# quang-ha/lammps-sph-multiphase

Hardware: AMD Instinct MI355X
Metric: particle-steps/s + achieved HBM GB/s, 1M-particle taitwater+rhosum, 1/2/4/8 GPUs (higher is better)
Workload: dtype f64

## Files before the change

### include/sph_hip.h

```cpp
#ifndef SPH_HIP_H
#define SPH_HIP_H

#include <stdint.h>

#ifdef __cplusplus
extern "C" {
#endif

#define SPH_HIP_ABI_VERSION 2

#define SPH_HIP_OK 0
#define SPH_HIP_EINVAL (-1)
#define SPH_HIP_ENODEV (-2)
#define SPH_HIP_ERUNTIME (-3)
#define SPH_HIP_ENOMEM (-4)
#define SPH_HIP_ECOMM (-5)
#define SPH_HIP_EOVERFLOW (-6)

#define SPH_LIST_FULL 0
#define SPH_LIST_HALF 1

#define SPH_VISC_MONAGHAN 0
#define SPH_VISC_MORRIS 1

// ... 129 lines not shown
  int kernel_path;
  const sph_engine_mp_config *mp;
} sph_engine_config;

typedef struct {
  int64_t step;
  int nlocal, nghost;
  int64_t nbr_full;
  int nbr_builds;
  int nbr_maxrow;
  int staged;
  int stage_max;
  double ms_rhosum, ms_tait, ms_heat, ms_integrate, ms_comm, ms_neigh;
  int64_t n_rhosum, n_tait, n_heat, n_neigh;
  int blk_nbig;
  int inner_rows;
  int inner_live;
  int flags;
  int64_t inner_refresh;
} sph_engine_stats;

#define SPH_STAT_RHO_FUSED (1 << 0)
#define SPH_STAT_BLK_R32 (1 << 1)
#define SPH_STAT_BLK_BIGIMG (1 << 2)
#define SPH_STAT_BLK_NOPRE (1 << 3)
#define SPH_STAT_BLK_ROWRETRY (1 << 4)
#define SPH_STAT_BLK_IMGRETRY (1 << 5)
#define SPH_STAT_MP_W4 (1 << 6)
#define SPH_STAT_MP_POW (1 << 7)
#define SPH_STAT_MP_ROW (1 << 8)
#define SPH_STAT_MP_RHO_LISTFILL (1 << 9)
#define SPH_STAT_CSORT_BINS (1 << 10)
#define SPH_STAT_CSORT_ROWS (1 << 11)

typedef struct sph_engine sph_engine;

int sph_engine_create(int device, const sph_engine_config *cfg, sph_engine **out);
int sph_engine_destroy(sph_engine *e);

int sph_engine_comm_uid(void *uid128);
int sph_engine_comm_init(sph_engine *e, const void *uid128, int nranks, int rank);
int sph_engine_comm_loopback(sph_engine *e, int on);
typedef struct sph_local_world sph_local_world;
int sph_local_world_create(int nranks, sph_local_world **out);
int sph_local_world_destroy(sph_local_world *w);
int sph_engine_comm_local(sph_engine *e, sph_local_world *w, int rank);
int sph_engine_comm_ipc(sph_engine *e, const char *name, int nranks, int rank, int mode);
#define SPH_TUNE_OVERLAP 1
#define SPH_TUNE_BLKUMF 2
#define SPH_TUNE_CSORT 3
int sph_engine_tune(sph_engine *e, int key, int value);
int sph_engine_csort_paths(sph_engine *e, int *mask);
int sph_engine_set_tags(sph_engine *e, const int *tags);

int sph_engine_set_atoms(sph_engine *e, int n, const double *x, const double *v,
                         const int *type, const double *rho, const double *en,
                         const double *cv);
int sph_engine_set_atoms_multiphase(sph_engine *e, const double *rmass, const double *cv,
                                    const double *cg);
int sph_engine_phase_change(sph_engine *e, const sph_phasechange_params *p, int nevery,
                            int seed);
int sph_engine_atom_sort(sph_engine *e, int sortfreq, double binsize);

int sph_engine_neigh_modify(sph_engine *e, int every, int delay, int check);

typedef struct {
  int64_t builds;
  int64_t dangerous;
  int64_t checks;
  int64_t last_build;
} sph_neigh_stats;
int sph_engine_neigh_stats(sph_engine *e, sph_neigh_stats *out);

typedef struct {
  int nevery;
  int minbound; double tmin;
  int maxbound; double tmax;
  double xmax;
  int type_mask;
} sph_dtreset;
int sph_engine_dt_reset(sph_engine *e, const sph_dtreset *fix);

typedef struct {
// ... 130 lines not shown
```

### lammps-sph-multiphase_amd/__init__.py

```python
from __future__ import annotations

import ctypes as C
import os

import numpy as np

HERE = os.path.dirname(os.path.abspath(__file__))
LIB_PATH = os.environ.get("SPH_HIP_LIB") or os.path.join(HERE, "libsph_hip.so")
HEADER = os.path.join(os.path.dirname(HERE), "include", "sph_hip.h")

SPH_LIST_FULL, SPH_LIST_HALF = 0, 1
SPH_VISC_MONAGHAN, SPH_VISC_MORRIS = 0, 1
SPH_MAXTYPES = 8
_NT2 = (SPH_MAXTYPES + 1) ** 2

ERRORS = {-1: "EINVAL", -2: "ENODEV", -3: "ERUNTIME", -4: "ENOMEM", -5: "ECOMM",
          -6: "EOVERFLOW"}


class HipError(RuntimeError):
    def __init__(self, code: int, msg: str):
        super().__init__(f"sph_hip {ERRORS.get(code, code)}: {msg}")
        self.code = code

# ... 856 lines not shown
            for c in classes:
                mask |= 1 << c
            _chk(self.L.sph_engine_set_timing(self.h, mask << 1))
        else:
            _chk(self.L.sph_engine_set_timing(self.h, 1 if on else 0))

    @property
    def nlocal(self):
        return self.L.sph_engine_nlocal(self.h)

    def get_atoms(self):
        n = self.nlocal
        out = {k: np.zeros((n, 3)) for k in ("x", "v", "f")}
        out.update({k: np.zeros(n) for k in ("rho", "e", "drho", "de")})
        out["tag"] = np.zeros(n, dtype=np.int32)
        _chk(self.L.sph_engine_get_atoms(self.h, out["x"].ctypes.data, out["v"].ctypes.data,
                                         out["rho"].ctypes.data, out["e"].ctypes.data,
                                         out["f"].ctypes.data, out["drho"].ctypes.data,
                                         out["de"].ctypes.data, out["tag"].ctypes.data))
        return out

    def set_tags(self, tags):
        tags = np.ascontiguousarray(tags, dtype=np.int32)
        _chk(self.L.sph_engine_set_tags(self.h, tags))

    def comm_local(self, world: "LocalWorld", rank: int):
        _chk(self.L.sph_engine_comm_local(self.h, world.h, rank))
        self._world = world

    def comm_init(self, uid: bytes, nranks: int, rank: int):
        buf = C.create_string_buffer(bytes(uid), 128)
        _chk(self.L.sph_engine_comm_init(self.h, buf, nranks, rank))

    TUNE_OVERLAP, TUNE_BLKUMF, TUNE_CSORT = 1, 2, 3

    def tune(self, key: int, value: int):
        _chk(self.L.sph_engine_tune(self.h, key, int(value)))

    IPC_DEVICE, IPC_HOST = 0, 1

    def comm_ipc(self, name: str, nranks: int, rank: int, mode: int = 0):
        _chk(self.L.sph_engine_comm_ipc(self.h, name.encode(), nranks, rank, int(mode)))

    def comm_loopback(self, on: bool = True):
        _chk(self.L.sph_engine_comm_loopback(self.h, 1 if on else 0))

    def neighbor_counts(self):
        c = np.zeros(self.nlocal, dtype=np.int32)
        _chk(self.L.sph_engine_neighbor_counts(self.h, c))
        return c

    STAT_RHO_FUSED, STAT_BLK_R32, STAT_BLK_BIGIMG = 1 << 0, 1 << 1, 1 << 2
    STAT_BLK_NOPRE, STAT_BLK_ROWRETRY, STAT_BLK_IMGRETRY = 1 << 3, 1 << 4, 1 << 5
    STAT_MP_W4, STAT_MP_POW, STAT_MP_ROW, STAT_MP_RHO_LISTFILL = 1 << 6, 1 << 7, 1 << 8, 1 << 9
    STAT_CSORT_BINS, STAT_CSORT_ROWS = 1 << 10, 1 << 11

    def csort_paths(self) -> int:
        m = _i(0)
        _chk(self.L.sph_engine_csort_paths(self.h, C.byref(m)))
        return m.value

    def stats(self) -> dict:
        s = EngineStats()
        _chk(self.L.sph_engine_stats_get(self.h, C.byref(s)))
        return s.as_dict()


def _moments_dict(count, mass, mx, mv, lo, hi, volume):
    d = dict(count=count, mass=mass, mx=mx, mv=mv, lo=lo, hi=hi, volume=volume)
    d["xcm"] = mx / mass if mass > 0.0 else np.zeros(3)
    d["vcm"] = mv / mass if mass > 0.0 else np.zeros(3)
    return d


def combine_moments(ranks):
    first = ranks[0]
    acc = {k: (first[k].copy() if isinstance(first[k], np.ndarray) else first[k])
           for k in ("count", "mass", "mx", "mv", "lo", "hi", "volume")}
    for r in ranks[1:]:
        for k in ("count", "mass", "mx", "mv", "volume"):
            acc[k] = acc[k] + r[k]
        acc["lo"] = np.minimum(acc["lo"], r["lo"])
        acc["hi"] = np.maximum(acc["hi"], r["hi"])
    return _moments_dict(**acc)


def gyration_dict(sums, mass):
    sums = np.array(sums, dtype=np.float64)
# ... 57 lines not shown
```

### lammps-sph-multiphase_amd/csrc/sph_blk_kernels.h

```cpp
#pragma once
#include <hip/hip_runtime.h>

#include <algorithm>
#include <type_traits>
#include <utility>

#include "sph_engine_kernels.h"
#include "sph_row2_kernels.h"
#include "sph_select.h"
#include "sph_util.h"

namespace sph {

constexpr int BLK_TPR = 16;

template <int BT>
__device__ __forceinline__ int blk_scan(int v, int *s_w, int *total) {
  const int lane = threadIdx.x & 63, w = threadIdx.x >> 6;
  int x = v;
#pragma unroll
  for (int d = 1; d < 64; d <<= 1) {
    const int y = __shfl_up(x, d, 64);
    if (lane >= d) x += y;
  }
// ... 968 lines not shown
      for (int p = tid; p < u; p += NTH)
        if ((s_bm[(p + 1) >> 5] >> ((p + 1) & 31)) & 1u)
          uilist[(size_t)b * ucap + rank(p + 1)] = ul[p];
    if (ren && tid == 0) {
      uicnt[b] = tot;
      if (umax) {
        atomicMax(umax, tot);
        atomicAdd(umax + 1, tot);
      }
    }
    const int grp = (tid & 63) / G;
    unsigned short *const out = snbi + (size_t)rr * sstride;
    int base = 0;
    sw.walk(c, lane, [&](int q, bool in) {
      const bool hit = hit_of(q, in);
      const unsigned long long m = __ballot(hit);
      const unsigned g = (unsigned)(m >> (grp * G)) & ((1u << G) - 1u);
      if (hit)
        out[blk_tpos<G, U>(base + __popc(g & ((1u << lane) - 1u)))] =
            (unsigned short)(ren ? blk_q(rank(blk_s<CQ>(q)) + 1, CQ) : q);
      base += __popc(g);
    });
    if (live) {
      if (lane == 0) {
        icnt[row] = base;
        if (x0) x0[row] = xi;
      }
      const int cend = min((base + U * G - 1) / (U * G) * (U * G), sstride);
      for (int k = base + lane; k < cend; k += G) out[blk_tpos<G, U>(k)] = 0;
    }
  }
}

#define SPH_BLK_FORCE_PARAMS                                                              \
  int n, const int *__restrict__ ulist, const int *__restrict__ ucnt, int ucap,                 \
      const unsigned short *__restrict__ snbr, int sstride, const int *__restrict__ rcnt,     \
      const double4 *__restrict__ xf, const double4 *__restrict__ vr,                         \
      const int *__restrict__ ty, const double *__restrict__ en,                              \
      const Coefs *__restrict__ cf, double4 *__restrict__ fo, double *__restrict__ de,        \
      double gx, double gy, double gz, int um, int cq,                                        \
      const unsigned short *__restrict__ snbi, const int *__restrict__ icnt,                  \
      const int *__restrict__ moved, const int *__restrict__ uilist,                          \
      const int *__restrict__ uicnt, const int *__restrict__ blist
#define SPH_BLK_FORCE_ARGS                                                                \
  n, ulist, ucnt, ucap, snbr, sstride, rcnt, xf, vr, ty, en, cf, fo, de, gx, gy, gz, um, cq, \
      snbi, icnt, moved, uilist, uicnt, blist
template <int R, int G, int U, int NCH, int VISC, int MODE, bool NT1, int EXP = 0, int AHEAD = 1>
__device__ __forceinline__ void blk_force_body(SPH_BLK_FORCE_PARAMS) {
  if (snbi && *moved == 0) {
    snbr = snbi;
    rcnt = icnt;
    ulist = uilist;
    ucnt = uicnt;
  }
  constexpr bool GAS = (MODE & M_GAS) != 0;
  constexpr bool TAIT = (MODE & (M_TAIT | M_GAS)) != 0;
  constexpr bool HEAT = (MODE & M_HEAT) != 0;
  constexpr bool EIMG = HEAT || GAS;
  constexpr int NTH = R * G;
  constexpr int CQ = (EIMG ? BLK_CHE : BLK_CH) / 16;
  constexpr bool FOLDV = TAIT && !HEAT && !GAS && NT1 && VISC == SPH_VISC_MONAGHAN;
  extern __shared__ __attribute__((aligned(16))) unsigned char blk_smem[];
  __shared__ TaitPair s_tp[(TAIT && !NT1) ? NT2 : 1];
  __shared__ HeatPair s_hp[(HEAT && !NT1) ? NT2 : 1];
  const int nt1 = cf->ntypes + 1;
  const int b = blist ? blist[xcd_block()] : (int)xcd_block();
  const int tid = threadIdx.x;
  const int u = EXP == 3 ? 0 : ucnt[b];
  const int nwin = u > um ? (u + um - 1) / um : 1;
  const int u0 = min(u, um);
  const int row = b * R + tid / G, lane = tid & (G - 1);
  const bool live = row < n;
  const int rr = live ? row : n - 1;
  const int c = live ? rcnt[rr] : 0;
  const int *const ul = ulist + (size_t)b * ucap;
  int jj[BLK_SP];
#pragma unroll
  for (int k = 0; k < BLK_SP; k++) jj[k] = tid + k * NTH < u0 ? ul[tid + k * NTH] : -1;
  BlkSlots<G, U, NCH> sw;
  sw.load(snbr + (size_t)rr * sstride, c, lane);
  const double4 xi = xf[rr];
// ... 139 lines not shown
  auto walk = [&](auto ld) {
    if constexpr (NCH > 0)
      blk_walk3<AHEAD>(sw, wave_max_count<G>(c), ld, pair);
    else
      sw.walk(c, lane, [&](int q, bool) { pair(ld(q)); });
  };
  if (nwin == 1) {
    walk(load);
  } else {
    const int qmax = blk_q(um, CQ);
    for (int w = 0; w < nwin; w++) {
      if (w > 0) {
        __syncthreads();
        stage(w, tid);
        __syncthreads();
      }
      const int qo = blk_q(w * um, CQ);
      walk([&](int q) {
        const int qq = q - qo;
        return load((unsigned)(qq - 1) < (unsigned)qmax ? qq : 0);
      });
    }
  }
  if (TAIT) {
    fx = group_sum<G>(fx);
    fy = group_sum<G>(fy);
    fz = group_sum<G>(fz);
    D = group_sum<G>(D);
    E = group_sum<G>(E);
  }
  if (HEAT) EH = group_sum<G>(EH);
  if (lane == 0 && live) {
    double dE = 0.0;
    if (TAIT) {
      const double g = NT1 ? t1.mm * t1.wK : 1.0;
      const double gd = NT1 ? t1.mj * t1.wK : 1.0;
      const double m = cf->mass[it];
      fo[row] = make_double4(g * fx + m * gx, g * fy + m * gy, g * fz + m * gz, gd * D);
      dE = -0.5 * (g * E);
    }
    if (HEAT) dE += NT1 ? (h1.hmD * h1.wK) * EH : EH;
    de[row] = dE;
  }
}

template <int R, int G, int U, int NCH, int VISC, int MODE, bool NT1, int EXP = 0>
__global__ void __launch_bounds__(R * G) k_blk_force(SPH_BLK_FORCE_PARAMS) {
  blk_force_body<R, G, U, NCH, VISC, MODE, NT1, EXP>(SPH_BLK_FORCE_ARGS);
}
template <int R, int G, int U, int NCH, int VISC, int MODE, bool NT1, int EXP = 0>
__global__ void __launch_bounds__(R * G) __attribute__((amdgpu_waves_per_eu(6, 6)))
k_blk_force_w6(SPH_BLK_FORCE_PARAMS) {
  blk_force_body<R, G, U, NCH, VISC, MODE, NT1, EXP, 0>(SPH_BLK_FORCE_ARGS);
}

static __global__ void k_blk_count_big(int nb, const int *__restrict__ ucnt, int um,
                                       int *__restrict__ nbig) {
  const int b = blockIdx.x * blockDim.x + threadIdx.x;
  if (b < nb && ucnt[b] > um) atomicAdd(nbig, 1);
}

static __global__ void __launch_bounds__(1024)
k_blk_stats(int nb, const int *__restrict__ ucnt, const int *__restrict__ kcnt,
            const int *__restrict__ uicnt, int *__restrict__ umax) {
  __shared__ int s_r[6][16];
  int v[6] = {0, 0, 0, 0, 0, 0};
  for (int b = threadIdx.x; b < nb; b += blockDim.x) {
    const int u = ucnt[b], k = kcnt[b], ui = uicnt ? uicnt[b] : 0;
    v[0] = max(v[0], u);
    v[1] = max(v[1], k);
    v[2] += k;
    v[3] += u;
    v[4] = max(v[4], ui);
    v[5] += ui;
  }
#pragma unroll
  for (int d = 32; d > 0; d >>= 1)
#pragma unroll
    for (int q = 0; q < 6; q++) {
      const int o = __shfl_xor(v[q], d, 64);
      v[q] = (q == 0 || q == 1 || q == 4) ? max(v[q], o) : v[q] + o;
    }
  const int w = threadIdx.x >> 6;
  if ((threadIdx.x & 63) == 0)
    for (int q = 0; q < 6; q++) s_r[q][w] = v[q];
  __syncthreads();
// ... 161 lines not shown
                         k.uilist, k.uicnt, k.blist);
    });
  });
}

struct BlkInnerRefresh {
  const int *cond = nullptr;
  int *zero = nullptr;
  double4 *x0 = nullptr;
  int *umax = nullptr;
};
inline void blk_inner(bool nt1, hipStream_t s, const BlkArgs &k, const double4 *xf,
                      const int *ty, const Coefs *cf, unsigned short *snbi, int *icnt,
                      const BlkInnerRefresh &rf = BlkInnerRefresh{}) {
  if (k.n == 0) return;
  blk_select(nt1, k, [&](auto sh, auto t, auto nch) {
    constexpr int R = sh.v[0], G = sh.v[1], U = sh.v[2], NCH = nch;
    constexpr bool NT1 = t;
    select_int<BLK_CHE / 16, BLK_CH / 16>(k.cq, [&](auto cq) {
      constexpr int CQ = cq;
      auto fn = k_blk_inner<R, G, U, NCH, NT1, CQ>;
      const size_t lds = blk_rho_lds(k.um, NT1);
      SPH_HIP_TRY(hipFuncSetAttribute((const void *)fn,
                                      hipFuncAttributeMaxDynamicSharedMemorySize, (int)lds));
      const int nb = blk_blocks(k.n, R);
      hipLaunchKernelGGL(fn, dim3(rf.cond ? std::min(nb, 512) : nb), dim3(R * G), lds, s, k.n,
                         k.ulist, k.ucnt, k.ucap, k.snbr, k.sstride, k.rcnt, xf, ty, cf, snbi,
                         icnt, k.um, rf.cond, rf.zero, rf.x0, k.uilist, k.uicnt, rf.umax);
    });
  });
}

inline void blk_force(bool nt1, int visc, int mode, hipStream_t s, const BlkArgs &k,
                      const RowArgs &a) {
  if (k.n == 0) return;
  const int visc1 = (visc == BLK_VISC_NONE && !nt1) ? SPH_VISC_MONAGHAN : visc;
  const int exp1 = nt1 ? k.exp : 0;
  blk_select(nt1, k, [&](auto sh, auto t, auto nch) {
    constexpr int R = sh.v[0], G = sh.v[1], U = sh.v[2], NCH = nch;
    constexpr bool NT1 = t;
    select_int<M_HEAT, M_TAIT, M_TAIT | M_HEAT, M_GAS>(mode, [&](auto m) {
      constexpr int MODE = m;
      select_int<SPH_VISC_MONAGHAN, SPH_VISC_MORRIS, BLK_VISC_NONE>(visc1, [&](auto vc) {
        constexpr int VISC = (MODE == M_TAIT || (vc == SPH_VISC_MORRIS && (MODE & M_TAIT)))
                                 ? (int)vc : SPH_VISC_MONAGHAN;
        auto launch = [&](auto ex) {
          constexpr int EXP = ex;
          auto fn = [] {
            if constexpr (NT1 && MODE == M_TAIT && EXP == 0 && NCH > 0)
              return k_blk_force_w6<R, G, U, NCH, VISC, MODE, NT1, EXP>;
            else
              return k_blk_force<R, G, U, NCH, VISC, MODE, NT1, EXP>;
          }();
          size_t lds = blk_lds(k.umf, k.cq, NT1);
#ifdef SPH_STUDY
          if (const char *e = getenv("SPH_LDS_PAD")) lds += (size_t)atoi(e);
#endif
          SPH_HIP_TRY(hipFuncSetAttribute(
              (const void *)fn, hipFuncAttributeMaxDynamicSharedMemorySize, (int)lds));
          const int nb = k.blist ? k.nlist : blk_blocks(k.n, R);
          if (nb == 0) return;
          hipLaunchKernelGGL(fn, dim3(nb), dim3(R * G), lds, s, k.n, k.ulist, k.ucnt, k.ucap,
                             k.snbr, k.sstride, k.rcnt, a.xf, a.vr, a.ty, a.en, a.cf, a.fo, a.de,
                             a.gx, a.gy, a.gz, k.umf, k.cq, k.snbi, k.icnt, k.moved, k.uilist,
                             k.uicnt, k.blist);
        };
        if constexpr (STUDY_BUILD && VISC == SPH_VISC_MONAGHAN && MODE == M_TAIT)
          select_int<0, 1, 2, 3>(exp1, launch);
        else
          launch(std::integral_constant<int, 0>{});
      });
    });
  });
}

}
```

### lammps-sph-multiphase_amd/csrc/sph_engine.hip

```cpp
#include <hip/hip_runtime.h>
#include <hipcub/hipcub.hpp>
#include <rocprofiler-sdk-roctx/roctx.h>

#include <algorithm>
#include <chrono>
#include <cstring>
#include <cmath>
#include <utility>
#include <vector>

#include "sph_coef.h"
#include "sph_comm.h"
#include "sph_dispatch.h"
#include "sph_blk_kernels.h"
#include "sph_engine_kernels.h"
#include "sph_engine_mp.h"
#include "sph_fix_kernels.h"
#include "sph_ipc.h"
#include "sph_moments_kernels.h"
#include "sph_mp2_kernels.h"
#include "sph_pc.h"
#include "sph_row2_kernels.h"
#include "sph_util.h"

// ... 1028 lines not shown
  st->nghost = e->nghost;
  st->nbr_full = e->list_entries();
  st->nbr_builds = e->nbr_builds;
  st->nbr_maxrow = e->nbr_maxrow;
  st->staged = e->blk ? 1 : 0;
  st->stage_max = e->blk ? e->blk_um : 0;
  st->ms_rhosum = e->ms[T_RHO];
  st->ms_tait = e->ms[T_TAIT];
  st->ms_heat = e->ms[T_HEAT];
  st->ms_integrate = e->ms[T_INT];
  st->ms_comm = e->ms[T_COMM];
  st->ms_neigh = e->ms[T_NEIGH];
  st->n_rhosum = e->nlaunch[T_RHO];
  st->n_tait = e->nlaunch[T_TAIT];
  st->n_heat = e->nlaunch[T_HEAT];
  st->n_neigh = e->nlaunch[T_NEIGH];
  st->blk_nbig = 0;
  if (e->blk && e->mx.p) {
    e->to_host(&st->blk_nbig, e->mx.p + 9, 1);
    SPH_HIP_TRY(hipStreamSynchronize(e->s));
  }
  st->inner_rows = e->inner ? 1 : 0;
  st->inner_live = 0;
  if (e->inner && e->moved.p) {
    int mv = 1;
    e->to_host(&mv, e->moved_flag(), 1);
    SPH_HIP_TRY(hipStreamSynchronize(e->s));
    st->inner_live = mv == 0 ? 1 : 0;
  }
  st->flags = (e->rho_fused_step >= 0 && e->rho_fused_step == e->step) ? SPH_STAT_RHO_FUSED : 0;
  if (e->blk) st->flags |= e->blk_flags;
  if (e->mp) st->flags |= e->mp_flags;
  if (e->blk || e->mp) st->flags |= e->cs_flags;
  st->inner_refresh = e->inner_refreshes;
  SPH_API_END
}

int sph_engine_set_timing(sph_engine *e, int on) {
  SPH_API_BEGIN
  SPH_REQUIRE(e, SPH_HIP_EINVAL, "sph_engine_set_timing: NULL engine");
  SPH_HIP_TRY(hipSetDevice(e->device));
  e->harvest();
  e->timing_mask = on == 1 ? (1 << T_NCLASS) - 1 : (on > 1 ? (on >> 1) & ((1 << T_NCLASS) - 1) : 0);
  e->timing = e->timing_mask != 0;
  for (int k = 0; k < T_NCLASS; k++) {
    e->ms[k] = 0.0;
    e->nlaunch[k] = 0;
  }
  SPH_API_END
}

int sph_engine_sync(sph_engine *e) {
  SPH_API_BEGIN
  SPH_REQUIRE(e, SPH_HIP_EINVAL, "sph_engine_sync: NULL engine");
  SPH_HIP_TRY(hipSetDevice(e->device));
  SPH_HIP_TRY(hipStreamSynchronize(e->s));
  SPH_API_END
}

int sph_engine_comm_uid(void *uid128) {
  SPH_API_BEGIN
  SPH_REQUIRE(uid128, SPH_HIP_EINVAL, "sph_engine_comm_uid: NULL buffer");
  static_assert(sizeof(ncclUniqueId) == 128, "ncclUniqueId is 128 bytes");
  ncclUniqueId id;
  SPH_NCCL_TRY(ncclGetUniqueId(&id));
  memcpy(uid128, &id, sizeof(id));
// ... 45 lines not shown
}

int sph_engine_comm_local(sph_engine *e, sph_local_world *w, int rank) {
  SPH_API_BEGIN
  SPH_REQUIRE(e && w, SPH_HIP_EINVAL, "sph_engine_comm_local: NULL argument");
  LocalWorld *lw = reinterpret_cast<LocalWorld *>(w);
  SPH_REQUIRE(rank >= 0 && rank < lw->n, SPH_HIP_EINVAL, "rank %d outside [0,%d)", rank, lw->n);
  attach(e, new LocalTransport(lw, rank));
  SPH_API_END
}

int sph_engine_comm_ipc(sph_engine *e, const char *name, int nranks, int rank, int mode) {
  SPH_API_BEGIN
  SPH_REQUIRE(e && name, SPH_HIP_EINVAL, "sph_engine_comm_ipc: NULL argument");
  SPH_HIP_TRY(hipSetDevice(e->device));
  attach(e, new IpcTransport(name, nranks, rank, mode, e->device));
  SPH_API_END
}

int sph_engine_tune(sph_engine *e, int key, int value) {
  SPH_API_BEGIN
  SPH_REQUIRE(e, SPH_HIP_EINVAL, "sph_engine_tune: NULL engine");
  SPH_REQUIRE(!e->setup_done, SPH_HIP_EINVAL, "sph_engine_tune: before sph_engine_setup");
  switch (key) {
    case SPH_TUNE_OVERLAP: e->overlap = value != 0; break;
    case SPH_TUNE_BLKUMF:
      SPH_REQUIRE(value >= 0, SPH_HIP_EINVAL, "sph_engine_tune: BLKUMF %d < 0", value);
      e->blkumf = value;
      break;
    case SPH_TUNE_CSORT:
      SPH_REQUIRE(value >= 0 && value <= 2, SPH_HIP_EINVAL, "sph_engine_tune: CSORT %d", value);
      e->csort = value;
      break;
    default: SPH_REQUIRE(false, SPH_HIP_EINVAL, "sph_engine_tune: unknown key %d", key);
  }
  SPH_API_END
}

int sph_engine_csort_paths(sph_engine *e, int *mask) {
  SPH_API_BEGIN
  SPH_REQUIRE(e && mask, SPH_HIP_EINVAL, "sph_engine_csort_paths: NULL argument");
  *mask = e->cs_flags;
  SPH_API_END
}

int sph_engine_set_tags(sph_engine *e, const int *tags) {
  SPH_API_BEGIN
  SPH_REQUIRE(e && (tags || e->nlocal == 0), SPH_HIP_EINVAL, "sph_engine_set_tags: bad argument");
  SPH_HIP_TRY(hipSetDevice(e->device));
  int mx = -1;
  for (int i = 0; i < e->nlocal; i++) {
    SPH_REQUIRE(tags[i] >= 0 && tags[i] < (1 << 30), SPH_HIP_EINVAL,
                "sph_engine_set_tags: tag %d outside [0, 2^30)", tags[i]);
    mx = std::max(mx, tags[i]);
  }
  if (e->nlocal)
    SPH_HIP_TRY(hipMemcpy(e->tag.p, tags, e->nlocal * sizeof(int), hipMemcpyHostToDevice));
  e->global_tags = true;
  e->tag_next = mx + 1;
  e->pc_tags_agreed = false;
  e->lidx_valid = false;
  SPH_API_END
}

int sph_engine_atom_sort(sph_engine *e, int sortfreq, double binsize) {
  SPH_API_BEGIN
// ... 9 lines not shown
```

### lammps-sph-multiphase_amd/csrc/sph_engine_kernels.h

```cpp
#pragma once
#include <hip/hip_runtime.h>
#include <hipcub/hipcub.hpp>

#include "sph_bins.h"
#include "sph_dispatch.h"
#include "sph_kernels.h"
#include "sph_mp2_kernels.h"

namespace sph {

struct StepConst {
  double dtv, dtf;
  double mass[MAXT + 1];
  int stationary_mask;
  const double4 *x0;
  double lim2;
  int *moved;
};

__device__ __forceinline__ void inner_check(const StepConst &sc, int i, const double4 &x) {
  if (!sc.x0) return;
  const double4 a = sc.x0[i];
  const double dx = x.x - a.x, dy = x.y - a.y, dz = x.z - a.z;
  if (dx * dx + dy * dy + dz * dz > sc.lim2) atomicOr(sc.moved, 1);
// ... 127 lines not shown
  const int i = blockIdx.x * blockDim.x + threadIdx.x;
  if (i >= n) return;
  const int t = ty[i];
  const double4 f = fo[i];
  if (!((sc.stationary_mask >> t) & 1)) {
    double4 v = vel[i];
    const double dtfm = step_dtf(sc, dr) / (rm ? rm[i] : sc.mass[t]);
    v.x += dtfm * f.x;
    v.y += dtfm * f.y;
    v.z += dtfm * f.z;
    vel[i] = v;
  }
  en[i] += step_dtf(sc, dr) * de[i];
  vr[i].w += step_dtf(sc, dr) * f.w;
}
static __global__ void k_final_integrate(int n, StepConst sc, double4 *__restrict__ vr,
                                         double *__restrict__ en, const int *__restrict__ ty,
                                         double4 *__restrict__ vel,
                                         const double4 *__restrict__ fo,
                                         const double *__restrict__ de,
                                         const double *__restrict__ rm) {
  final_integrate(n, sc, vr, en, ty, vel, fo, de, rm, DtFrom<false>{});
}
static __global__ void k_final_integrate_dt(int n, StepConst sc, double4 *__restrict__ vr,
                                            double *__restrict__ en,
                                            const int *__restrict__ ty,
                                            double4 *__restrict__ vel,
                                            const double4 *__restrict__ fo,
                                            const double *__restrict__ de,
                                            const double *__restrict__ rm, DtFrom<true> dr) {
  final_integrate(n, sc, vr, en, ty, vel, fo, de, rm, dr);
}

template <bool CHK, bool DTR>
static __global__ void k_final_initial(int n, StepConst sc, double4 *__restrict__ xf,
                                       double4 *__restrict__ vr, double *__restrict__ en,
                                       const int *__restrict__ ty, double4 *__restrict__ vel,
                                       const double4 *__restrict__ fo,
                                       const double *__restrict__ de,
                                       const double *__restrict__ rm, StepOpt<CHK, DTR> nh) {
  const int i = blockIdx.x * blockDim.x + threadIdx.x;
  if (i >= n) return;
  bool mv = false;
  const int t = ty[i];
  double4 vv = vr[i];
  const double4 f = fo[i];
  const double dei = de[i];
  double e = en[i];
  e += step_dtf(sc, nh) * dei;
  vv.w += step_dtf(sc, nh) * f.w;
  e += step_dtf(sc, nh) * dei;
  vv.w += step_dtf(sc, nh) * f.w;
  if (!((sc.stationary_mask >> t) & 1)) {
    double4 x = xf[i];
    double4 v = vel[i];
    const double dtfm = step_dtf(sc, nh) / (rm ? rm[i] : sc.mass[t]);
    v.x += dtfm * f.x;
    v.y += dtfm * f.y;
    v.z += dtfm * f.z;
    vv.x = v.x + 2.0 * dtfm * f.x;
    vv.y = v.y + 2.0 * dtfm * f.y;
    vv.z = v.z + 2.0 * dtfm * f.z;
    v.x += dtfm * f.x;
    v.y += dtfm * f.y;
    v.z += dtfm * f.z;
    x.x += step_dtv(sc, nh) * v.x;
    x.y += step_dtv(sc, nh) * v.y;
    x.z += step_dtv(sc, nh) * v.z;
    vel[i] = v;
    xf[i] = x;
    inner_check(sc, i, x);
    if (CHK) mv = neigh_moved(nh, i, x);
  }
  en[i] = e;
  vr[i] = vv;
  if (CHK) neigh_raise(nh, mv);
}

struct DtFix {
  int minbound, maxbound;
  double tmin, tmax, xmax, ftm2v;
  int type_mask;
};
struct DtRecord {
  double dtv, dtf;
  double dt, atime;
  long long atimestep, laststep, changes;
  double brick_min;
};
constexpr double DT_BIG = 1.0e20;

__device__ __forceinline__ double dt_reset_atom(double vx, double vy, double vz, double fx,
                                                double fy, double fz, double m, double xmax,
                                                double ftm2v) {
#pragma clang fp contract(off)
  const double massinv = 1.0 / m;
  const double vsq = vx * vx + vy * vy + vz * vz;
  const double fsq = fx * fx + fy * fy + fz * fz;
  double dtv = DT_BIG, dtf = DT_BIG;
  if (vsq > 0.0) dtv = xmax / __builtin_sqrt(vsq);
  if (fsq > 0.0) dtf = __builtin_sqrt(2.0 * xmax / (ftm2v * __builtin_sqrt(fsq) * massinv));
// ... 852 lines not shown
```

### lammps-sph-multiphase_amd/csrc/sph_engine_state.h

```cpp
#pragma once

namespace sph {
#ifndef SPH_INNER_FRAC
#define SPH_INNER_FRAC 0.0625
#endif
int g_alloc_log = 0;
static int env_int(const char *name, int dflt) {
  const char *s = getenv(name);
  return s ? atoi(s) : dflt;
}
#ifdef SPH_STUDY
static int study_int(const char *name, int dflt) { return env_int(name, dflt); }
#else
static int study_int(const char *, int dflt) { return dflt; }
#endif
int row2_tile() {
  static int t = study_int("SPH_ROW2TILE", 3);
  return t;
}
}
static int morton_div() {
  static int v = std::max(1, study_int("SPH_MORTON_DIV", 4));
  return v;
}
// ... 102 lines not shown
  DBuf<int> pf_idx, pf_idx2;
  DBuf<long long> pf_cnt;
  DBuf<double> pf_sum;
  DBuf<double> mom_buf;
  bool pc_tags_agreed = false;
  std::vector<double> cv_by_tag;

  int nlocal = 0, nghost = 0;
  int pg[3] = {1, 1, 1}, myloc[3] = {0, 0, 0}, procneigh[3][2] = {{0, 0}, {0, 0}, {0, 0}};
  int me = 0, nprocs = 1;
  Transport *tr = nullptr;
  struct Swap {
    int dim = 0, dir = 0, sendproc = 0, recvproc = 0, nsend = 0, nrecv = 0, firstrecv = 0;
    int pbc = 0;
    double lo = 0.0, hi = 0.0, shift = 0.0;
    double lo_sel = 0.0, hi_sel = 0.0;
    bool remote = false;
    DBuf<int> list;
  };
  Swap swaps[6];
  int nswap = 0;
  DBuf<unsigned char> cbs, cbr, flag2;
  DBuf<int> sel2;
  bool loopback = false;
  bool multi() const { return pg[0] * pg[1] * pg[2] > 1 || loopback; }
  hipStream_t s2 = nullptr;
  hipEvent_t ev_fork = nullptr, ev_join = nullptr;
  DBuf<int> rows_in, rows_bd;
  DBuf<unsigned char> fl_in, fl_bd;
  int n_in = 0, n_bd = 0;
  bool ov_ready = false;
  bool overlap = false;
  int blkumf = 0;
  int64_t step = 0;
  int64_t rho_fused_step = -1;
  int64_t last_sort = 0;
  bool force_sort = false;
  bool setup_done = false;
  bool global_tags = false;
  int last_build = 0;
  bool nm_set = false, nm_check = false;
  int nm_every = 1, nm_delay = 0;
  int64_t nm_ago = 0, nm_builds = 0, nm_danger = 0, nm_checks = 0;
  DBuf<double4> xhold;
  DBuf<int> nm_flag;
  int *h_nm = nullptr;
  bool dtr_on = false;
  int dtr_nevery = 1;
  DtFix dtr{};
  DBuf<DtRecord> dt_rec;
  DBuf<double> dt_part;
  DtRecord *h_dt = nullptr;

  DBuf<double4> xf, vr;
  DBuf<double> en;
  DBuf<int> ty;
  DBuf<double4> vel, fo;
  DBuf<double> de;
  DBuf<int> tag;
  DBuf<double4> xf2, vr2, vel2;
  DBuf<double> en2;
  DBuf<int> ty2, tag2;
  DBuf<int> gowner, gimg;
  DBuf<int> gorank, goidx;
  bool dr_ok = false;
  std::vector<int> dr_peer;
// ... 131 lines not shown
  bool blk_args_pre(const BlkShape &sh) const;
  BlkArgs blk_args() const;
  void build_all(bool need_csr);
  void build_inner();
  int *moved_flag() const;
  void refresh_inner(bool rebuild_next);
  void rebuild();
  int neigh_every() const { return nm_set ? nm_every : (cfg.neigh_every > 0 ? cfg.neigh_every : 1); }
  bool neigh_eligible(int64_t ago) const;
  void neigh_built();
  bool neigh_flag_any();

  void hole_fill(int n, int nl, int nst);
  void atom_sort();
  void lidx_from_tags();
  void pc_ghost_slots();
  void pc_rank_swap(int ns, int first, int bits);
  void pc_ghost_slots_multi();
  void phase_change();

  bool overlap_on() const;
  void classify_rows();
  void fork();
  void join();
  void pair_compute_overlap();
  void dt_reset_init();
  void dt_end_of_step(bool with_final);
  RowArgs row_args();
  ForceArgs force_args();
  int64_t list_span() const;
  int64_t list_entries();
  Row2Args row2_args();
  bool use_row2() const { return row2_fits((long)nlocal + nghost, (long)list_span()); }
  void pair_compute(bool do_rhosum, bool setup = false);
  void setup_forces_full();
  static dim3 mp_rows(int rows) { return dim3((unsigned)(((long long)rows * 8 + 255) / 256)); }
  void pair_compute_mp();
  double uniform_cv(const char *who) const;
  void post_force_setmeso();
  StepMass type_mass() const;
  void post_force_forcefix();
  bool rhosum_due() const;
  void setup();
  void launch_integrate(bool first, bool chk);
  void run(int nsteps);
};

inline hipEvent_t sph_engine::get_ev() {
  if (!evpool.empty()) {
    hipEvent_t e = evpool.back();
    evpool.pop_back();
    return e;
  }
  hipEvent_t e;
  SPH_HIP_TRY(hipEventCreate(&e));
  return e;
}
inline sph_engine::Scope::Scope(sph_engine *eng, int cls)
    : e(eng), on(((eng->timing_mask >> cls) & 1) != 0) {
  static const char *const bucket[T_NCLASS] = {"Pair:rhosum", "Pair:taitwater",
                                               "Pair:heatconduction", "Modify:integrate",
                                               "Comm", "Neigh"};
  roctxRangePushA(bucket[cls]);
  if (!on) return;
  p.a = e->get_ev();
  p.b = e->get_ev();
  p.cls = cls;
// ... 86 lines not shown
```

### lammps-sph-multiphase_amd/csrc/sph_engine_step.h

```cpp
#pragma once
#include "sph_engine_state.h"

inline bool sph_engine::overlap_on() const {
  return multi() && overlap && (blk || use_row2()) && (force_mode & M_TAIT) != 0 &&
         cfg.rhosum_nstep > 0;
}
inline void sph_engine::classify_rows() {
  const int n = nlocal;
  if (!s2) {
    SPH_HIP_TRY(hipStreamCreateWithFlags(&s2, hipStreamNonBlocking));
    SPH_HIP_TRY(hipEventCreateWithFlags(&ev_fork, hipEventDisableTiming));
    SPH_HIP_TRY(hipEventCreateWithFlags(&ev_join, hipEventDisableTiming));
  }
  if (blk) {
    const int nb = blk_blocks(n, blk_shape(blk_sh).R);
    fl_in.reserve_min1(nb);
    fl_bd.reserve_min1(nb);
    if (nb)
      hipLaunchKernelGGL(k_blk_interior, dim3(nb), dim3(64), 0, s, nb, ulist.p, ucnt.p,
                         BLK_UCAP, nlocal, fl_in.p, fl_bd.p);
    n_in = select_flagged(fl_in.p, nb, rows_in);
    n_bd = select_flagged(fl_bd.p, nb, rows_bd);
    SPH_REQUIRE(n_in + n_bd == nb, SPH_HIP_ERUNTIME, "block classification lost blocks");
    ov_ready = true;
// ... 155 lines not shown
  return a;
}
inline int64_t sph_engine::list_span() const {
  return strided ? (int64_t)nlocal * list_stride : nbr_total;
}
inline int64_t sph_engine::list_entries() {
  if (!strided) return nbr_total;
  if (nlocal == 0) return 0;
  blen.reserve(1);
  cub([&](void *t, size_t &tb) {
    return hipcub::DeviceReduce::Sum(t, tb, ccnt.p, blen.p, nlocal, s);
  });
  long long v = 0;
  to_host(&v, blen.p, 1);
  SPH_HIP_TRY(hipStreamSynchronize(s));
  return v;
}
inline Row2Args sph_engine::row2_args() {
  Row2Args b;
  b.a = row_args();
  b.nall = nlocal + nghost;
  b.ntot = (int)list_span();
  if (strided) {
    b.stride = list_stride;
    b.rcnt = ccnt.p;
  }
  b.lp = row2_lp();
  b.iv = strided && list_perm_g > 0 && list_perm_g == row2_iv_g();
  b.exp = row2_exp();
  b.tbits = strided && list_tbits;
  return b;
}

inline void sph_engine::pair_compute(bool do_rhosum, bool setup) {
  if (mp) {
    pair_compute_mp();
    return;
  }
  const int nall = nlocal + nghost;
  if (do_rhosum) {
    {
      Scope t(this, T_RHO);
      if (blk) {
        blk_rhosum(nt1(), s, blk_args(), xf.p, ty.p, vr.p, dc);
      } else if (use_row2()) {
        row2_rhosum(nt1(), s, row2_args());
      } else {
        RhoArgs ra{nlocal, nullptr, off.p, nbr.p, xf.p, ty.p, vr.p, nullptr, dc};
        launch_rhosum(cfg.dim, true, nt1(), s, ra);
      }
    }
    if (multi()) {
      Scope t(this, T_COMM);
      forward_rho_multi();
    } else if (nghost) {
      Scope t(this, T_COMM);
      launch(k_forward_rho, nghost, nghost, nlocal, gowner.p, xf.p, vr.p);
    }
  } else if (force_mode & M_TAIT) {
    launch(k_eos, nall, nall, xf.p, vr.p, ty.p, dc);
  }
  if ((force_mode & M_GAS) && nall)
    launch(k_eos_gas, nall, nall, xf.p, vr.p, en.p, ty.p, dc);
  if (force_mode && setup) {
    setup_forces_full();
  } else if (force_mode && blk) {
    Scope t(this, force_class());
    blk_force(nt1(), blk_visc(), force_mode, s, blk_args(), row_args());
  } else if (force_mode && use_row2()) {
    Scope t(this, force_class());
    row2_force(nt1(), row_visc(), force_mode, s, row2_args());
  } else if (force_mode) {
    Scope t(this, force_class());
    launch_force(cfg.dim, nt1(), s, row_visc(), force_mode, force_args());
  } else {
    SPH_HIP_TRY(hipMemsetAsync(fo.p, 0, nlocal * sizeof(double4), s));
    SPH_HIP_TRY(hipMemsetAsync(de.p, 0, nlocal * sizeof(double), s));
  }
}

inline void sph_engine::setup_forces_full() {
  const int n = nlocal, nall = nlocal + nghost;
  if (force_mode == 0 || n == 0) return;
  vsg.reserve_min1(nghost);
  if (nghost)
    dev_copy(vsg.p, vr.p + n, (size_t)nghost);
  forward();
  fo.reserve(nall, true, s);
  de.reserve(nall, true, s);
  ForceArgs a = force_args();
  a.vso = vso.p;
  a.vsg = vsg.p;
  launch_force(cfg.dim, nt1(), s, row_visc(), force_mode, a);
}

inline void sph_engine::pair_compute_mp() {
  const int n = nlocal, nall = nlocal + nghost;
  fo.reserve_min1(n, true, s);
// ... 179 lines not shown
  post_force_forcefix();
  nm_builds = nm_danger = nm_checks = 0;
  neigh_built();
  if (dtr_on) {
    dt_reset_init();
    dt_end_of_step(false);
  }
  setup_done = true;
}

inline void sph_engine::launch_integrate(bool first, bool chk) {
  Scope t(this, T_INT);
  select_bool(chk, [&](auto c) {
    constexpr bool CHK = c;
    select_bool(dtr_on, [&](auto d) {
      constexpr bool DTR = d;
      StepOpt<CHK, DTR> o{};
      if constexpr (CHK) {
        o.xhold = xhold.p;
        o.trig2 = 0.25 * cfg.skin * cfg.skin;
        o.flag = nm_flag.p;
      }
      if constexpr (DTR) o.rec = &dt_rec.p->dtv;
      if (first)
        launch((k_initial_integrate<CHK, DTR>), nlocal, nlocal, sc, xf.p, vr.p, en.p, ty.p, vel.p,
               fo.p, de.p, rm.p, o);
      else
        launch((k_final_initial<CHK, DTR>), nlocal, nlocal, sc, xf.p, vr.p, en.p, ty.p, vel.p,
               fo.p, de.p, rm.p, o);
    });
  });
}

inline void sph_engine::run(int nsteps) {
  bool final_done = false;
  for (int k = 0; k < nsteps; k++) {
    step++;
    if (sc.x0) sc.moved = moved_flag();
    const bool pc_due = pc && step == pc_next;
    const bool elig = !pc_due && neigh_eligible(nm_ago + 1);
    const bool chk = elig && nm_check;
    launch_integrate(dtr_on ? (k == 0 || final_done) : k == 0, chk);
    bool build = pc_due;
    if (!pc_due) {
      nm_ago++;
      if (chk) {
        nm_checks++;
        build = neigh_flag_any();
        if (build && nm_ago == std::max(neigh_every(), nm_delay)) nm_danger++;
      } else {
        build = elig;
      }
    }
    if (pc_due) {
      phase_change();
      pc_next += pc_nevery;
    }
    if (build) {
      rebuild();
      neigh_built();
      pair_compute(rhosum_due());
    } else if (ov_ready && rhosum_due() && overlap_on()) {
      pair_compute_overlap();
    } else {
      forward();
      pair_compute(rhosum_due());
    }
    post_force_setmeso();
    post_force_forcefix();
    refresh_inner(nm_check ? (pc && step + 1 == pc_next) : (!pc && neigh_eligible(nm_ago + 1)));
    if (timing && pending.size() > 4096) harvest();
    final_done = dtr_on && step % dtr_nevery == 0;
    if (final_done) dt_end_of_step(true);
  }
  if (nsteps > 0 && !final_done) {
    Scope t(this, T_INT);
    if (dtr_on)
      launch(k_final_integrate_dt, nlocal, nlocal, sc, vr.p, en.p, ty.p, vel.p, fo.p, de.p, rm.p,
             DtFrom<true>{&dt_rec.p->dtv});
    else
      launch(k_final_integrate, nlocal, nlocal, sc, vr.p, en.p, ty.p, vel.p, fo.p, de.p, rm.p);
  }
  SPH_HIP_TRY(hipGetLastError());
}
```

Measured before the change: 1.850 billion.

## Fuse final/initial integrate into taitwater blocked force kernel epilogue

Adds a FUSE template path to the blocked force kernel so the per-atom final+initial Verlet integrate runs in the force epilogue. The force and de arrays are no longer written and re-read, and a separate integrate launch per step is skipped. New positions and velocities go into double-buffered xf2/vr2 arrays that are then swapped, so neighbours still read the old positions while the kernel runs. The path is enabled by default only for single-GPU, taitwater-only, blocked-list runs with no fixes, no neighbour check and no dt reset. It adds register pressure to the force kernel and extra state-ordering complexity around refresh_inner.

```diff
diff --git a/include/sph_hip.h b/include/sph_hip.h
--- a/include/sph_hip.h
+++ b/include/sph_hip.h
@@ -185,6 +185,7 @@
 #define SPH_STAT_MP_RHO_LISTFILL (1 << 9)
 #define SPH_STAT_CSORT_BINS (1 << 10)
 #define SPH_STAT_CSORT_ROWS (1 << 11)
+#define SPH_STAT_FUSEINT (1 << 12)
 
 typedef struct sph_engine sph_engine;
 
@@ -202,6 +203,7 @@
 #define SPH_TUNE_OVERLAP 1
 #define SPH_TUNE_BLKUMF 2
 #define SPH_TUNE_CSORT 3
+#define SPH_TUNE_FUSEINT 4
 int sph_engine_tune(sph_engine *e, int key, int value);
 int sph_engine_csort_paths(sph_engine *e, int *mask);
 int sph_engine_set_tags(sph_engine *e, const int *tags);
diff --git a/lammps-sph-multiphase_amd/__init__.py b/lammps-sph-multiphase_amd/__init__.py
--- a/lammps-sph-multiphase_amd/__init__.py
+++ b/lammps-sph-multiphase_amd/__init__.py
@@ -912,7 +912,7 @@
         buf = C.create_string_buffer(bytes(uid), 128)
         _chk(self.L.sph_engine_comm_init(self.h, buf, nranks, rank))
 
-    TUNE_OVERLAP, TUNE_BLKUMF, TUNE_CSORT = 1, 2, 3
+    TUNE_OVERLAP, TUNE_BLKUMF, TUNE_CSORT, TUNE_FUSEINT = 1, 2, 3, 4
 
     def tune(self, key: int, value: int):
         _chk(self.L.sph_engine_tune(self.h, key, int(value)))
@@ -934,6 +934,7 @@
     STAT_BLK_NOPRE, STAT_BLK_ROWRETRY, STAT_BLK_IMGRETRY = 1 << 3, 1 << 4, 1 << 5
     STAT_MP_W4, STAT_MP_POW, STAT_MP_ROW, STAT_MP_RHO_LISTFILL = 1 << 6, 1 << 7, 1 << 8, 1 << 9
     STAT_CSORT_BINS, STAT_CSORT_ROWS = 1 << 10, 1 << 11
+    STAT_FUSEINT = 1 << 12
 
     def csort_paths(self) -> int:
         m = _i(0)
diff --git a/lammps-sph-multiphase_amd/csrc/sph_blk_kernels.h b/lammps-sph-multiphase_amd/csrc/sph_blk_kernels.h
--- a/lammps-sph-multiphase_amd/csrc/sph_blk_kernels.h
+++ b/lammps-sph-multiphase_amd/csrc/sph_blk_kernels.h
@@ -1024,6 +1024,15 @@
   }
 }
 
+template <bool FUSE>
+struct BlkFuse {};
+template <>
+struct BlkFuse<true> {
+  StepConst sc;
+  double4 *xn, *vn;
+  double4 *vel;
+  double *en;
+};
 #define SPH_BLK_FORCE_PARAMS                                                              \
   int n, const int *__restrict__ ulist, const int *__restrict__ ucnt, int ucap,                 \
       const unsigned short *__restrict__ snbr, int sstride, const int *__restrict__ rcnt,     \
@@ -1033,12 +1042,14 @@
       double gx, double gy, double gz, int um, int cq,                                        \
       const unsigned short *__restrict__ snbi, const int *__restrict__ icnt,                  \
       const int *__restrict__ moved, const int *__restrict__ uilist,                          \
-      const int *__restrict__ uicnt, const int *__restrict__ blist
+      const int *__restrict__ uicnt, const int *__restrict__ blist, BlkFuse<FUSE> fu
 #define SPH_BLK_FORCE_ARGS                                                                \
   n, ulist, ucnt, ucap, snbr, sstride, rcnt, xf, vr, ty, en, cf, fo, de, gx, gy, gz, um, cq, \
-      snbi, icnt, moved, uilist, uicnt, blist
-template <int R, int G, int U, int NCH, int VISC, int MODE, bool NT1, int EXP = 0, int AHEAD = 1>
+      snbi, icnt, moved, uilist, uicnt, blist, fu
+template <int R, int G, int U, int NCH, int VISC, int MODE, bool NT1, int EXP = 0, int AHEAD = 1,
+          bool FUSE = false>
 __device__ __forceinline__ void blk_force_body(SPH_BLK_FORCE_PARAMS) {
+  static_assert(!FUSE || (MODE == M_TAIT && EXP == 0), "FUSE: taitwater alone");
   if (snbi && *moved == 0) {
     snbr = snbi;
     rcnt = icnt;
@@ -1244,26 +1255,45 @@
   if (HEAT) EH = group_sum<G>(EH);
   if (lane == 0 && live) {
     double dE = 0.0;
+    double4 f = make_double4(0.0, 0.0, 0.0, 0.0);
     if (TAIT) {
       const double g = NT1 ? t1.mm * t1.wK : 1.0;
       const double gd = NT1 ? t1.mj * t1.wK : 1.0;
       const double m = cf->mass[it];
-      fo[row] = make_double4(g * fx + m * gx, g * fy + m * gy, g * fz + m * gz, gd * D);
+      f = make_double4(g * fx + m * gx, g * fy + m * gy, g * fz + m * gz, gd * D);
       dE = -0.5 * (g * E);
     }
     if (HEAT) dE += NT1 ? (h1.hmD * h1.wK) * EH : EH;
-    de[row] = dE;
-  }
-}
-
-template <int R, int G, int U, int NCH, int VISC, int MODE, bool NT1, int EXP = 0>
+    if constexpr (FUSE) {
+      const StepConst &sc = fu.sc;
+      const bool moving = !((sc.stationary_mask >> it) & 1);
+      double4 x = xi, vv = vi, v = make_double4(0.0, 0.0, 0.0, 0.0);
+      if (FOLDV) vv.w = vr[row].w;
+      double e = fu.en[row];
+      if (moving) v = fu.vel[row];
+      final_initial_atom(sc.dtv, sc.dtf, sc.mass[it], moving, f, dE, x, v, vv, e);
+      if (moving) {
+        fu.vel[row] = v;
+        inner_check(sc, row, x);
+      }
+      fu.xn[row] = x;
+      fu.vn[row] = vv;
+      fu.en[row] = e;
+    } else {
+      if (TAIT) fo[row] = f;
+      de[row] = dE;
+    }
+  }
+}
+
+template <int R, int G, int U, int NCH, int VISC, int MODE, bool NT1, int EXP = 0, bool FUSE = false>
 __global__ void __launch_bounds__(R * G) k_blk_force(SPH_BLK_FORCE_PARAMS) {
-  blk_force_body<R, G, U, NCH, VISC, MODE, NT1, EXP>(SPH_BLK_FORCE_ARGS);
-}
-template <int R, int G, int U, int NCH, int VISC, int MODE, bool NT1, int EXP = 0>
+  blk_force_body<R, G, U, NCH, VISC, MODE, NT1, EXP, 1, FUSE>(SPH_BLK_FORCE_ARGS);
+}
+template <int R, int G, int U, int NCH, int VISC, int MODE, bool NT1, int EXP = 0, bool FUSE = false>
 __global__ void __launch_bounds__(R * G) __attribute__((amdgpu_waves_per_eu(6, 6)))
 k_blk_force_w6(SPH_BLK_FORCE_PARAMS) {
-  blk_force_body<R, G, U, NCH, VISC, MODE, NT1, EXP, 0>(SPH_BLK_FORCE_ARGS);
+  blk_force_body<R, G, U, NCH, VISC, MODE, NT1, EXP, 0, FUSE>(SPH_BLK_FORCE_ARGS);
 }
 
 static __global__ void k_blk_count_big(int nb, const int *__restrict__ ucnt, int um,
@@ -1491,8 +1521,10 @@
 }
 
 inline void blk_force(bool nt1, int visc, int mode, hipStream_t s, const BlkArgs &k,
-                      const RowArgs &a) {
+                      const RowArgs &a, const BlkFuse<true> *fuse = nullptr) {
   if (k.n == 0) return;
+  SPH_REQUIRE(!fuse || (mode == M_TAIT && (!nt1 || k.exp == 0)), SPH_HIP_EINVAL,
+              "blk_force: the fused integrate exists for taitwater alone (mode %d)", mode);
   const int visc1 = (visc == BLK_VISC_NONE && !nt1) ? SPH_VISC_MONAGHAN : visc;
   const int exp1 = nt1 ? k.exp : 0;
   blk_select(nt1, k, [&](auto sh, auto t, auto nch) {
@@ -1503,14 +1535,17 @@
       select_int<SPH_VISC_MONAGHAN, SPH_VISC_MORRIS, BLK_VISC_NONE>(visc1, [&](auto vc) {
         constexpr int VISC = (MODE == M_TAIT || (vc == SPH_VISC_MORRIS && (MODE & M_TAIT)))
                                  ? (int)vc : SPH_VISC_MONAGHAN;
-        auto launch = [&](auto ex) {
+        auto launch = [&](auto ex, auto fz) {
           constexpr int EXP = ex;
+          constexpr bool FUSE = decltype(fz)::value && MODE == M_TAIT && EXP == 0;
           auto fn = [] {
             if constexpr (NT1 && MODE == M_TAIT && EXP == 0 && NCH > 0)
-              return k_blk_force_w6<R, G, U, NCH, VISC, MODE, NT1, EXP>;
+              return k_blk_force_w6<R, G, U, NCH, VISC, MODE, NT1, EXP, FUSE>;
             else
-              return k_blk_force<R, G, U, NCH, VISC, MODE, NT1, EXP>;
+              return k_blk_force<R, G, U, NCH, VISC, MODE, NT1, EXP, FUSE>;
           }();
+          BlkFuse<FUSE> fu{};
+          if constexpr (FUSE) fu = *fuse;
           size_t lds = blk_lds(k.umf, k.cq, NT1);
 #ifdef SPH_STUDY
           if (const char *e = getenv("SPH_LDS_PAD")) lds += (size_t)atoi(e);
@@ -1522,12 +1557,14 @@
           hipLaunchKernelGGL(fn, dim3(nb), dim3(R * G), lds, s, k.n, k.ulist, k.ucnt, k.ucap,
                              k.snbr, k.sstride, k.rcnt, a.xf, a.vr, a.ty, a.en, a.cf, a.fo, a.de,
                              a.gx, a.gy, a.gz, k.umf, k.cq, k.snbi, k.icnt, k.moved, k.uilist,
-                             k.uicnt, k.blist);
+                             k.uicnt, k.blist, fu);
         };
-        if constexpr (STUDY_BUILD && VISC == SPH_VISC_MONAGHAN && MODE == M_TAIT)
-          select_int<0, 1, 2, 3>(exp1, launch);
-        else
-          launch(std::integral_constant<int, 0>{});
+        select_bool(fuse != nullptr, [&](auto fz) {
+          if constexpr (STUDY_BUILD && VISC == SPH_VISC_MONAGHAN && MODE == M_TAIT)
+            select_int<0, 1, 2, 3>(exp1, [&](auto ex) { launch(ex, fz); });
+          else
+            launch(std::integral_constant<int, 0>{}, fz);
+        });
       });
     });
   });
diff --git a/lammps-sph-multiphase_amd/csrc/sph_engine.hip b/lammps-sph-multiphase_amd/csrc/sph_engine.hip
--- a/lammps-sph-multiphase_amd/csrc/sph_engine.hip
+++ b/lammps-sph-multiphase_amd/csrc/sph_engine.hip
@@ -1084,6 +1084,7 @@
   if (e->blk) st->flags |= e->blk_flags;
   if (e->mp) st->flags |= e->mp_flags;
   if (e->blk || e->mp) st->flags |= e->cs_flags;
+  st->flags |= e->fuse_flag;
   st->inner_refresh = e->inner_refreshes;
   SPH_API_END
 }
@@ -1195,6 +1196,10 @@
       SPH_REQUIRE(value >= 0 && value <= 2, SPH_HIP_EINVAL, "sph_engine_tune: CSORT %d", value);
       e->csort = value;
       break;
+    case SPH_TUNE_FUSEINT:
+      SPH_REQUIRE(value == 0 || value == 1, SPH_HIP_EINVAL, "sph_engine_tune: FUSEINT %d", value);
+      e->fuseint = value != 0;
+      break;
     default: SPH_REQUIRE(false, SPH_HIP_EINVAL, "sph_engine_tune: unknown key %d", key);
   }
   SPH_API_END
diff --git a/lammps-sph-multiphase_amd/csrc/sph_engine_kernels.h b/lammps-sph-multiphase_amd/csrc/sph_engine_kernels.h
--- a/lammps-sph-multiphase_amd/csrc/sph_engine_kernels.h
+++ b/lammps-sph-multiphase_amd/csrc/sph_engine_kernels.h
@@ -183,6 +183,30 @@
   final_integrate(n, sc, vr, en, ty, vel, fo, de, rm, dr);
 }
 
+__device__ __forceinline__ void final_initial_atom(double dtv, double dtf, double m, bool moving,
+                                                   const double4 &f, double dei, double4 &x,
+                                                   double4 &v, double4 &vv, double &e) {
+  e += dtf * dei;
+  vv.w += dtf * f.w;
+  e += dtf * dei;
+  vv.w += dtf * f.w;
+  if (moving) {
+    const double dtfm = dtf / m;
+    v.x += dtfm * f.x;
+    v.y += dtfm * f.y;
+    v.z += dtfm * f.z;
+    vv.x = v.x + 2.0 * dtfm * f.x;
+    vv.y = v.y + 2.0 * dtfm * f.y;
+    vv.z = v.z + 2.0 * dtfm * f.z;
+    v.x += dtfm * f.x;
+    v.y += dtfm * f.y;
+    v.z += dtfm * f.z;
+    x.x += dtv * v.x;
+    x.y += dtv * v.y;
+    x.z += dtv * v.z;
+  }
+}
+
 template <bool CHK, bool DTR>
 static __global__ void k_final_initial(int n, StepConst sc, double4 *__restrict__ xf,
                                        double4 *__restrict__ vr, double *__restrict__ en,
@@ -198,26 +222,16 @@
   const double4 f = fo[i];
   const double dei = de[i];
   double e = en[i];
-  e += step_dtf(sc, nh) * dei;
-  vv.w += step_dtf(sc, nh) * f.w;
-  e += step_dtf(sc, nh) * dei;
-  vv.w += step_dtf(sc, nh) * f.w;
-  if (!((sc.stationary_mask >> t) & 1)) {
-    double4 x = xf[i];
-    double4 v = vel[i];
-    const double dtfm = step_dtf(sc, nh) / (rm ? rm[i] : sc.mass[t]);
-    v.x += dtfm * f.x;
-    v.y += dtfm * f.y;
-    v.z += dtfm * f.z;
-    vv.x = v.x + 2.0 * dtfm * f.x;
-    vv.y = v.y + 2.0 * dtfm * f.y;
-    vv.z = v.z + 2.0 * dtfm * f.z;
-    v.x += dtfm * f.x;
-    v.y += dtfm * f.y;
-    v.z += dtfm * f.z;
-    x.x += step_dtv(sc, nh) * v.x;
-    x.y += step_dtv(sc, nh) * v.y;
-    x.z += step_dtv(sc, nh) * v.z;
+  const bool moving = !((sc.stationary_mask >> t) & 1);
+  double4 x = make_double4(0.0, 0.0, 0.0, 0.0), v = x;
+  double m = 1.0;
+  if (moving) {
+    x = xf[i];
+    v = vel[i];
+    m = rm ? rm[i] : sc.mass[t];
+  }
+  final_initial_atom(step_dtv(sc, nh), step_dtf(sc, nh), m, moving, f, dei, x, v, vv, e);
+  if (moving) {
     vel[i] = v;
     xf[i] = x;
     inner_check(sc, i, x);
diff --git a/lammps-sph-multiphase_amd/csrc/sph_engine_state.h b/lammps-sph-multiphase_amd/csrc/sph_engine_state.h
--- a/lammps-sph-multiphase_amd/csrc/sph_engine_state.h
+++ b/lammps-sph-multiphase_amd/csrc/sph_engine_state.h
@@ -158,6 +158,8 @@
   bool ov_ready = false;
   bool overlap = false;
   int blkumf = 0;
+  bool fuseint = true;
+  int fuse_flag = 0;
   int64_t step = 0;
   int64_t rho_fused_step = -1;
   int64_t last_sort = 0;
@@ -355,7 +357,8 @@
   int64_t list_entries();
   Row2Args row2_args();
   bool use_row2() const { return row2_fits((long)nlocal + nghost, (long)list_span()); }
-  void pair_compute(bool do_rhosum, bool setup = false);
+  void pair_compute(bool do_rhosum, bool setup = false, bool fuse = false);
+  bool fuse_step() const;
   void setup_forces_full();
   static dim3 mp_rows(int rows) { return dim3((unsigned)(((long long)rows * 8 + 255) / 256)); }
   void pair_compute_mp();
diff --git a/lammps-sph-multiphase_amd/csrc/sph_engine_step.h b/lammps-sph-multiphase_amd/csrc/sph_engine_step.h
--- a/lammps-sph-multiphase_amd/csrc/sph_engine_step.h
+++ b/lammps-sph-multiphase_amd/csrc/sph_engine_step.h
@@ -211,7 +211,7 @@
   return b;
 }
 
-inline void sph_engine::pair_compute(bool do_rhosum, bool setup) {
+inline void sph_engine::pair_compute(bool do_rhosum, bool setup, bool fuse) {
   if (mp) {
     pair_compute_mp();
     return;
@@ -243,6 +243,20 @@
     launch(k_eos_gas, nall, nall, xf.p, vr.p, en.p, ty.p, dc);
   if (force_mode && setup) {
     setup_forces_full();
+  } else if (force_mode && blk && fuse) {
+    Scope t(this, force_class());
+    xf2.reserve_exact(xf.cap);
+    vr2.reserve_exact(vr.cap);
+    BlkFuse<true> fu;
+    fu.sc = sc;
+    fu.sc.moved = sc.x0 ? moved.p + ((step + 1) & 1) : nullptr;
+    fu.xn = xf2.p;
+    fu.vn = vr2.p;
+    fu.vel = vel.p;
+    fu.en = en.p;
+    blk_force(nt1(), blk_visc(), force_mode, s, blk_args(), row_args(), &fu);
+    std::swap(xf, xf2);
+    std::swap(vr, vr2);
   } else if (force_mode && blk) {
     Scope t(this, force_class());
     blk_force(nt1(), blk_visc(), force_mode, s, blk_args(), row_args());
@@ -488,15 +502,22 @@
   });
 }
 
+inline bool sph_engine::fuse_step() const {
+  return fuseint && blk && !multi() && !mp && force_mode == M_TAIT && !pc && !nm_check &&
+         !dtr_on && sm.nfix == 0 && ff.nfix == 0 && row2_exp() == 0;
+}
+
 inline void sph_engine::run(int nsteps) {
   bool final_done = false;
+  bool fused = false;
+  fuse_flag = 0;
   for (int k = 0; k < nsteps; k++) {
     step++;
     if (sc.x0) sc.moved = moved_flag();
     const bool pc_due = pc && step == pc_next;
     const bool elig = !pc_due && neigh_eligible(nm_ago + 1);
     const bool chk = elig && nm_check;
-    launch_integrate(dtr_on ? (k == 0 || final_done) : k == 0, chk);
+    if (!fused) launch_integrate(dtr_on ? (k == 0 || final_done) : k == 0, chk);
     bool build = pc_due;
     if (!pc_due) {
       nm_ago++;
@@ -512,19 +533,25 @@
       phase_change();
       pc_next += pc_nevery;
     }
+    auto refresh = [&] {
+      refresh_inner(nm_check ? (pc && step + 1 == pc_next) : (!pc && neigh_eligible(nm_ago + 1)));
+    };
     if (build) {
       rebuild();
       neigh_built();
-      pair_compute(rhosum_due());
-    } else if (ov_ready && rhosum_due() && overlap_on()) {
+    }
+    fused = k + 1 < nsteps && fuse_step();
+    if (!build && !fused && ov_ready && rhosum_due() && overlap_on()) {
       pair_compute_overlap();
     } else {
-      forward();
-      pair_compute(rhosum_due());
-    }
+      if (!build) forward();
+      if (fused) refresh();
+      pair_compute(rhosum_due(), false, fused);
+    }
+    if (fused) fuse_flag = SPH_STAT_FUSEINT;
     post_force_setmeso();
     post_force_forcefix();
-    refresh_inner(nm_check ? (pc && step + 1 == pc_next) : (!pc && neigh_eligible(nm_ago + 1)));
+    if (!fused) refresh();
     if (timing && pending.size() > 4096) harvest();
     final_done = dtr_on && step % dtr_nevery == 0;
     if (final_done) dt_end_of_step(true);
```

Result: faster. 1.880 billion, median of 6 (+1.6%).
